# OpenDriveLab/ThinkTwice

Hardware: AMD Instinct MI355X
Metric: frames/sec forward (4-cam+LiDAR, thinktwice.py cfg) (higher is better)
Workload: dtype bf16x3h; 1 GPU; forward_inference thinktwice.py cfg: 8 frames x (2 sweeps x 4 cams x 448x896 + 65536-pt LiDAR), ResNet50+PAFPN+DepthNet+UNet+LSS splat, LidarNet, fusion, 5-stage decoder; parallelism=replicas x1 (no data-path collective), launch=eager launches, 3 batches in flight on alternating streams, batches_in_flight=3

## Files before the change

### include/thinktwice_hip.h

```cpp
#ifndef THINKTWICE_HIP_H
#define THINKTWICE_HIP_H

#include <stddef.h>
#include <stdint.h>

#ifdef __cplusplus
extern "C" {
#endif

#define TT_F32 0
#define TT_BF16 1
#define TT_F16 2

#define TT_ACT_NONE 0
#define TT_ACT_RELU 1
#define TT_ACT_SIGMOID 2
#define TT_ACT_GELU 3
#define TT_ACT_SOFTPLUS 4
#define TT_ACT_SOFTPLUS_CLAMP 5

const char* tt_last_error(void);
const char* tt_conv_last_kernel(void);
int tt_conv_set_trace(void* stamps_or_null);
int tt_version(void);
// ... 61 lines not shown
    int act;
    int dtype;
    int out_dtype;
    const int* gather_idx;
    const int* m_dev;
    float* splitk_ws;
    const void* weight_x3;
    const int* row_perm;
    const unsigned* row_mask;
    int splitk_slices;
    int in_pair, out_pair;
    const void* weight_h2;
    float* out2; int out2_cstride, out2_coff;
    int res1_up_h, res1_up_w;
    int res1_f32;
} tt_conv_desc;

int tt_conv2d_fwd(const tt_conv_desc* d, void* stream);
int tt_conv2d_splitk_slices(const tt_conv_desc* d);
int tt_conv2d_plan(const tt_conv_desc* d, char* label, int label_bytes);

int tt_seg_feedback_chain(const float* x, long long R, int x_stride, int K1, const float* w1, const float* scale1,
                          const float* shift1, int act1, const float* w2, const void* w2_x3, int N2, const float* scale2,
                          const float* shift2, int act2, float* out, int out_stride, int out_coff, void* stream);

typedef struct tt_chain_stage {
    const void* w; const float* bias;
    int K, Kp, N, act, in_sel;
    const float* res; int res_stride, res_coff;
    const float* side; const float* side_w; int side_stride, side_k;
// ... 362 lines not shown
```

### thinktwice_amd/build.py

```python
import os
import subprocess
import sys
from concurrent.futures import ThreadPoolExecutor

from . import _lib

HERE = os.path.dirname(os.path.abspath(__file__))
CSRC = os.path.join(HERE, "csrc")
OBJ = os.path.join(CSRC, "_obj")
LIB = os.path.join(HERE, "libthinktwice_hip.so")
HIPCC = os.environ.get("HIPCC", "/opt/rocm/bin/hipcc")
FLAGS = ["--offload-arch=gfx950", "-O3", "-std=c++17", "-fPIC", "-munsafe-fp-atomics", "-ffp-contract=off",
         "-Wno-unused-result"]


EXTRA_FLAGS = {"conv_x3_pipe.hip": ["-fno-slp-vectorize"]}


def _sources():
    return sorted(f for f in os.listdir(CSRC) if f.endswith((".hip", ".cpp")))


def _deps_mtime():
    hdrs = [os.path.join(CSRC, f) for f in os.listdir(CSRC) if f.endswith((".h", ".inc"))]
    hdrs.append(os.path.join(HERE, "..", "include", "thinktwice_hip.h"))
    hdrs.append(os.path.abspath(__file__))
    return max(os.path.getmtime(h) for h in hdrs)


def _compile(src, hdr_mtime, verbose):
    obj = os.path.join(OBJ, src + ".o")
# ... 81 lines not shown
```

### thinktwice_amd/csrc/conv_choose.cpp

```cpp
#include <stdint.h>

#include "conv_choose.h"

namespace tt {
namespace {

bool aligned16(const void* p) { return (reinterpret_cast<uintptr_t>(p) & 15) == 0; }

void set_tile(ConvChoice* c, int family, int bn, int waves_m, int waves_n, int bkb, int stages) {
    c->family = family;
    c->bn = bn;
    c->waves_m = waves_m;
    c->waves_n = waves_n;
    c->bkb = bkb;
    c->stages = stages;
}

bool choose_h2(const ConvArgs& a, ConvChoice* c) {
    if (a.gather || a.m_dev || a.ws || a.pixel_shuffle2 || a.Cin % 64 != 0 || a.KH * a.KW > 31 || a.K < 64) return false;
    static const bool pipe = env_flag("TT_H2_PIPE", true);
    if (pipe && a.Cout % 128 == 0 && a.K >= 1152) set_tile(c, CONV_H2_PIPE, 128, 4, 1, 128, 32);
    else if (a.Cout > 64) set_tile(c, CONV_H2, 128, 4, 2, 128, 32);
    else set_tile(c, CONV_H2, 64, 8, 1, 128, 33);
    return true;
// ... 104 lines not shown
    static const bool pipe = env_flag("TT_X3_PIPE", true);
    if (pipe && a.K >= 1152 && bn != 64 && x3_pipe_ok(a, bn)) {
        static const bool run3 = env_flag("TT_X3_RUN3", true);
        const bool runs = run3 && a.KW == 3 && a.KH <= 5 && a.stride == 1 && a.dil == 1 && a.pad == 1 && a.OH == a.H && a.OW == a.W &&
                          (a.N == 1 || a.in_nstride == (long long)a.H * a.W * a.in_cstride);
        set_tile(c, runs ? CONV_X3_RUN3 : CONV_X3_PIPE, bn, 4, 1, 128, 23);
    } else if (bn == 256) {
        set_tile(c, CONV_GLDS, 256, 4, 2, 128, 23);
    } else {
        set_tile(c, CONV_GLDS, bn, 8, 1, 128, 2);
    }
    if (bn == 256) c->main_rows = main_rows;
    return true;
}

bool choose_glds(const ConvArgs& a, int dtype, ConvChoice* c) {
    constexpr int min_tiles = 2;
    if (a.gather) {
        const bool cin_ok = a.Cin >= 16 && (a.Cin & (a.Cin - 1)) == 0;
        if (dtype == TT_F32 || !cin_ok || a.M < 2048 || a.Cout < 16 || a.Cout > 128) return false;
        if (a.Cout <= 32) set_tile(c, CONV_GLDS, 32, 8, 1, 128, 2);
        else if (a.Cout <= 64) set_tile(c, CONV_GLDS, 64, 8, 1, 128, 2);
        else set_tile(c, CONV_GLDS, 128, 4, 2, 128, 2);
        c->gather = true;
        return true;
    }
    if (a.m_dev || a.M < 2048 || a.Cout < 64 || a.KH * a.KW > 32) return false;
    if (dtype == TT_F32) {
        if (a.Cin % 16 != 0 || div_up(a.K, 16) < min_tiles) return false;
        if (a.Cout > 64) set_tile(c, CONV_GLDS, 128, 4, 2, 64, 3);
// ... 43 lines not shown
        if (a.ws_slices > 0) {
            const int eff = div_up(nk, div_up(nk, c->splits));
            TT_REQUIRE(a.ws_slices >= eff, "tt_conv2d_fwd: split-K workspace holds %d slices, %d needed", a.ws_slices, eff);
            c->slices = eff;
        }
    }
    return 0;
}

}

int conv_choose(const ConvArgs& a, const ConvFacts& f, ConvChoice* c) {
    *c = ConvChoice{};
    c->splits = 1;
    const bool ws = a.ws || f.assume_ws;
    if (f.weight_h2) {
        TT_REQUIRE(aligned16(f.weight_h2), "tt_conv2d_fwd: weight_h2 must be 16-byte aligned");
        TT_REQUIRE(choose_h2(a, c), "tt_conv2d_fwd: weight_h2 layer outside the h2 kernel's contract (Cin=%d KH*KW=%d)", a.Cin,
                   a.KH * a.KW);
        return 0;
    }
    TT_REQUIRE(!f.out2 || a.vec_epi, "tt_conv2d_fwd: out2 needs the vector epilogue (aligned channel counts)");
    TT_REQUIRE(!f.res1_up || a.vec_epi, "tt_conv2d_fwd: an upsampled res1 needs the vector epilogue (aligned channel counts)");
    TT_REQUIRE(!f.res1_f32 || (a.vec_epi && a.res_vec), "tt_conv2d_fwd: an f32 res1 needs the vector epilogue and aligned residual rows");
    TT_REQUIRE(!(f.dtype == TT_F32 && a.out_dtype != TT_F32 && a.res1) || (a.vec_epi && a.res_vec),
               "tt_conv2d_fwd: a 16-bit output of an f32 layer with a residual needs the vector epilogue");
    if (a.flags & (32 | 64)) {
        TT_REQUIRE(a.vec_epi && aligned16(f.weight_x3) && a.K % 16 == 0,
                   "tt_conv2d_fwd: in_pair / out_pair need the vector epilogue and a 16-byte aligned weight_x3");
        TT_REQUIRE(choose_x3(a, c), "tt_conv2d_fwd: pair-format layer outside the LDS-DMA bf16x3 kernel's contract (M=%d Cin=%d Cout=%d)",
// ... 23 lines not shown
    return t;
}

void conv_label(const ConvChoice& c, int dtype, char* out, size_t bytes) {
    const char* tn = dtype == TT_F32 ? "float" : "16-bit";
    const char* pre = c.apair ? " pre-split A" : "";
    const char* tail = c.main_rows > 0 ? " + tail" : "";
    switch (c.family) {
        case CONV_H2: snprintf(out, bytes, "conv_h2_kernel<%d, %d, %d, %d, %d>", c.bn, c.waves_m, c.waves_n, c.stages / 10, c.stages % 10); break;
        case CONV_H2_PIPE: snprintf(out, bytes, "conv_h2_pipe_kernel"); break;
        case CONV_SMALL: snprintf(out, bytes, "conv_small_kernel"); break;
        case CONV_SP_RUNS_L2: snprintf(out, bytes, "sp_conv_runs_l2_kernel<%d>", c.bkb / 4); break;
        case CONV_SP_RUNS: snprintf(out, bytes, "sp_conv_runs_kernel<%d, %d, %d>", c.bn / (32 * c.waves_n), c.waves_m, c.waves_n); break;
        case CONV_X3_PIPE: snprintf(out, bytes, "conv_x3_pipe_kernel<%s>%s%s", c.bn == 128 ? "4, 1, 128" : "4, 1", pre, tail); break;
        case CONV_X3_RUN3: snprintf(out, bytes, "conv_x3_run3_kernel<%d>%s%s", c.bn, pre, tail); break;
        case CONV_GLDS:
            snprintf(out, bytes, "conv_igemm_glds_kernel<%s, %d, %d, %d, %d, %d, %s, %s>%s%s", tn, c.bn, c.waves_m, c.waves_n, c.bkb,
                     c.stages, c.gather ? "true" : "false", c.x3 ? "true" : "false", pre, c.splits > 1 ? " split-K" : tail);
            break;
        default: snprintf(out, bytes, "conv_igemm_kernel<%s, 128, %d>%s", tn, c.bn, c.splits > 1 ? " split-K" : ""); break;
    }
}

}
```

### thinktwice_amd/csrc/conv_choose.h

```cpp
#pragma once
#include <stddef.h>

#include "tt_common.h"

namespace tt {

struct ConvArgs {
    const void* in;
    const void* weight;
    void* out;
    const float* scale;
    const float* shift;
    const float* shift_n;
    const void* res1;
    const void* res2;
    const int* gather;
    const int* m_dev;
    const int* row_perm;
    const unsigned* row_mask;
    float* ws;
    long long in_nstride, out_nstride;
    int N, H, W, Cin, in_cstride, in_coff;
    int Cout, KH, KW, stride, pad, dil;
    int OH, OW, out_cstride, out_coff;
// ... 12 lines not shown
    int flags;
    int res1_up_h, res1_up_w;
    float* out2;
    int out2_cstride, out2_coff;
    long long* trace;
};

enum ConvFamily {
    CONV_H2,
    CONV_H2_PIPE,
    CONV_SMALL,
    CONV_SP_RUNS_L2,
    CONV_SP_RUNS,
    CONV_X3_PIPE,
    CONV_X3_RUN3,
    CONV_GLDS,
    CONV_IGEMM,
};

constexpr int kSpL2MinRows = 16384;

struct ConvFacts {
    int dtype;
    const void* weight_x3;
    const void* weight_h2;
    bool out2, res1_up, res1_f32;
    bool assume_ws;
};

struct ConvChoice {
// ... 15 lines not shown
```

### thinktwice_amd/csrc/conv_common.h

```cpp
#pragma once
#include <type_traits>
#include "conv_choose.h"

namespace tt {
extern thread_local char g_conv_kernel[96];
extern long long* g_conv_trace;


typedef float f32x16 __attribute__((ext_vector_type(16)));
typedef __bf16 bf16x8 __attribute__((ext_vector_type(8)));
typedef _Float16 f16x8 __attribute__((ext_vector_type(8)));

template <typename T> struct Mfma;
template <> struct Mfma<float> {
    __device__ static __forceinline__ void run(const uint4& a, const uint4& b, f32x16& c) {
        c = __builtin_amdgcn_mfma_f32_32x32x2f32(__uint_as_float(a.x), __uint_as_float(b.x), c, 0, 0, 0);
        c = __builtin_amdgcn_mfma_f32_32x32x2f32(__uint_as_float(a.y), __uint_as_float(b.y), c, 0, 0, 0);
        c = __builtin_amdgcn_mfma_f32_32x32x2f32(__uint_as_float(a.z), __uint_as_float(b.z), c, 0, 0, 0);
        c = __builtin_amdgcn_mfma_f32_32x32x2f32(__uint_as_float(a.w), __uint_as_float(b.w), c, 0, 0, 0);
    }
};
template <> struct Mfma<uint16_t> {
    __device__ static __forceinline__ void run(const uint4& a, const uint4& b, f32x16& c) {
        c = __builtin_amdgcn_mfma_f32_32x32x16_bf16(__builtin_bit_cast(bf16x8, a),
// ... 381 lines not shown
            if (p.out_dtype == TT_F32)
                reinterpret_cast<float*>(p.out)[o] = v;
            else
                store16(p.out, o, v, p.out_dtype);
            if (p.out2) p.out2[(long long)mo * p.out2_cstride + p.out2_coff + co] = v;
        }
    }
}

int launch_conv_h2(const ConvChoice& c, ConvArgs& a, hipStream_t st);
int launch_conv_small(ConvArgs& a, int dtype, hipStream_t st);
int launch_sp_conv_l2(const ConvChoice& c, ConvArgs& a, hipStream_t st);
int launch_sp_conv_runs(const ConvChoice& c, ConvArgs& a, hipStream_t st);
int launch_conv_x3_pipe(const ConvChoice& c, ConvArgs& a, hipStream_t st);
int launch_conv_glds(const ConvChoice& c, ConvArgs& a, int dtype, hipStream_t st);

}
```

### thinktwice_amd/csrc/conv_igemm.hip

```cpp
#include <stdlib.h>

#include "conv_common.h"

namespace tt {

template <typename T, int BM, int BN, int WAVES_M, int WAVES_N, bool GATHER, int KX = 1>
__global__ __launch_bounds__(256) void conv_igemm_kernel(const ConvArgs p) {
    constexpr int VEC = Elem<T>::kVec;
    constexpr int BKB = ((sizeof(T) == 4) ? 64 : 128) * KX;
    constexpr int BK = BKB / (int)sizeof(T);
    constexpr int VPR = BKB / 16;
    constexpr int ROWB = BKB + 16;
    constexpr int NVA = (BM * VPR + 255) / 256;
    constexpr int NVB = (BN * VPR + 255) / 256;
    constexpr int WTM = BM / WAVES_M, WTN = BN / WAVES_N;
    constexpr int TM = WTM / 32, TN = WTN / 32;
    static_assert(WAVES_M * WAVES_N == 4, "4 waves");

    extern __shared__ __attribute__((aligned(16))) unsigned char smem[];
    const int nbuf = (p.K > BK) ? 2 : 1;
    unsigned char* sA = smem;
    unsigned char* sB = smem + nbuf * BM * ROWB;

    const int tid = threadIdx.x;
// ... 305 lines not shown
               "tt_conv2d_fwd: residuals are not supported with pixel_shuffle2");
    a.tiles_n = 1; a.cin_fast = 0; a.m_begin = 0;
    a.trace = g_conv_trace;
    a.flags = 16;
    if (d->in_pair || d->out_pair) {
        TT_REQUIRE(d->dtype == TT_F32 && d->out_dtype == TT_F32 && d->weight_x3 && !d->gather_idx && !d->splitk_ws && !d->pixel_shuffle2,
                   "tt_conv2d_fwd: in_pair / out_pair go with dense bf16x3 layers (f32 containers, weight_x3, no split-K workspace)");
        TT_REQUIRE(!d->out_pair || (!d->res1 && !d->res2 && !d->shift_n && d->Cout % 16 == 0 && d->out_cstride % 16 == 0 &&
                                    d->out_coff % 16 == 0 && (reinterpret_cast<uintptr_t>(d->out) & 63) == 0),
                   "tt_conv2d_fwd: out_pair needs Cout / out_cstride / out_coff multiples of 16, a 64-byte aligned output and no "
                   "residual / per-image shift");
        if (d->in_pair) a.flags |= 32;
        if (d->out_pair) a.flags |= 64;
    }
    if (d->res1_f32) a.flags |= 128;
    {
        const int co_vec = (d->out_dtype == TT_F32 && !d->out_pair) ? 4 : 8;
        const int osz = d->out_dtype == TT_F32 ? 4 : 2;
        const int cr = d->pixel_shuffle2 ? d->Cout / 4 : d->Cout;
        bool ok = (cr % co_vec == 0) && (d->out_cstride % co_vec == 0) && (d->out_coff % co_vec == 0) &&
                  (a.out_nstride % co_vec == 0) && ((reinterpret_cast<uintptr_t>(d->out) & 15) == 0);
        (void)osz;
        a.vec_epi = ok ? 1 : 0;
        auto res_ok = [&](const void* r, int cs, int co_) {
            return !r || ((cs % co_vec == 0) && (co_ % co_vec == 0) && ((reinterpret_cast<uintptr_t>(r) & 15) == 0));
        };
        a.res_vec = (res_ok(d->res1, d->res1_cstride, d->res1_coff) && res_ok(d->res2, d->res2_cstride, d->res2_coff)) ? 1 : 0;
    }
    f.dtype = d->dtype;
    f.weight_x3 = d->weight_x3;
// ... 28 lines not shown
            r = launch_conv_small(a, d->dtype, st);
            break;
        case CONV_SP_RUNS_L2:
            what = "tt_conv2d_fwd(sp l2)";
            r = launch_sp_conv_l2(c, a, st);
            break;
        case CONV_SP_RUNS:
            what = "tt_conv2d_fwd(glds x3)";
            r = launch_sp_conv_runs(c, a, st);
            break;
        case CONV_X3_PIPE:
        case CONV_X3_RUN3:
            what = pair ? "tt_conv2d_fwd(glds x3, pair)" : "tt_conv2d_fwd(glds x3)";
            r = launch_conv_x3_pipe(c, a, st);
            break;
        case CONV_GLDS:
            what = !c.x3 ? "tt_conv2d_fwd(glds)" : c.splits > 1 ? "tt_conv2d_fwd(glds x3 split-K)" : pair ? "tt_conv2d_fwd(glds x3, pair)" : "tt_conv2d_fwd(glds x3)";
            if (c.splits > 1) a.ws_slices = c.slices;
            r = launch_conv_glds(c, a, d->dtype, st);
            break;
        default:
            a.row_perm = nullptr;
            a.row_mask = nullptr;
            r = launch_conv_igemm(c, a, d->dtype, st);
            break;
    }
    if (r < 0) return r;
    conv_label(c, d->dtype, g_conv_kernel, sizeof(g_conv_kernel));
    if (c.main_rows > 0) {
        ConvArgs t = a;
        t.m_begin = c.main_rows * 256;
        if (launch_conv_glds(conv_tail_choice(c), t, d->dtype, st) < 0) return -1;
    }
    if (c.splits > 1) launch_splitk_finalize(a, d->dtype, st);
    return check_launch(what);
}

extern "C" int tt_conv2d_splitk_slices(const tt_conv_desc* d) {
    ConvArgs a;
    ConvFacts f;
    ConvChoice c;
    if (conv2d_prepare(d, a, f)) return 0;
    if (d->in_pair || d->out_pair || d->weight_h2 || d->res1_up_w > 0) return 0;
    f.assume_ws = true;
    if (conv_choose(a, f, &c)) return 0;
    return c.splits > 1 ? c.slices : 0;
}

extern "C" int tt_conv2d_plan(const tt_conv_desc* d, char* label, int label_bytes) {
    ConvArgs a;
    ConvFacts f;
    ConvChoice c;
    if (const int r = conv2d_prepare(d, a, f)) return r;
    if (const int r = conv_choose(a, f, &c)) return r;
    TT_REQUIRE(label && label_bytes > 0, "tt_conv2d_plan: no room for the label");
    conv_label(c, d->dtype, label, (size_t)label_bytes);
    return 0;
}
// ... 1 lines not shown
```

### thinktwice_amd/csrc/elementwise.hip

```cpp
#include "tt_common.h"

namespace tt {

template <typename T> struct Vec;
template <> struct Vec<float> {
    static constexpr int N = 4;
    float v[4];
    __device__ __forceinline__ void load(const float* p) {
        const float4 t = *reinterpret_cast<const float4*>(p);
        v[0] = t.x; v[1] = t.y; v[2] = t.z; v[3] = t.w;
    }
    __device__ __forceinline__ void store(float* p) const {
        *reinterpret_cast<float4*>(p) = make_float4(v[0], v[1], v[2], v[3]);
    }
};
template <typename T16> struct Vec16 {
    static constexpr int N = 8;
    float v[8];
    __device__ __forceinline__ void load(const T16* p) {
        const uint4 t = *reinterpret_cast<const uint4*>(p);
        const uint32_t w[4] = {t.x, t.y, t.z, t.w};
#pragma unroll
        for (int i = 0; i < 4; ++i) Pair16<T16>::unpack(w[i], v[2 * i], v[2 * i + 1]);
    }
// ... 132 lines not shown
        b.load(base + ((long long)y0 * W + x1) * C);
        cc.load(base + ((long long)y1 * W + x0) * C);
        d.load(base + ((long long)y1 * W + x1) * C);
#pragma unroll
        for (int k = 0; k < V; ++k) {
            const float top = (1.f - lx) * a.v[k] + lx * b.v[k];
            const float bot = (1.f - lx) * cc.v[k] + lx * d.v[k];
            o.v[k] = (1.f - ly) * top + ly * bot;
        }
        o.store(out + i * V);
    }
}

__global__ void bilinear_up2_ac_pair_kernel(const float* __restrict__ in, float* __restrict__ out, int N, int H, int W, int C) {
    const int cv = C / 8, OH = 2 * H, OW = 2 * W;
    const float sh = (OH > 1) ? (float)(H - 1) / (float)(OH - 1) : 0.f;
    const float sw = (OW > 1) ? (float)(W - 1) / (float)(OW - 1) : 0.f;
    const long long total = (long long)N * OH * OW * cv;
    TT_GRID_STRIDE(i, total) {
        const int c = (int)(i % cv);
        long long r = i / cv;
        const int ox = (int)(r % OW); r /= OW;
        const int oy = (int)(r % OH);
        const long long n = r / OH;
        const float fy = sh * oy, fx = sw * ox;
        const int y0 = (int)fy, x0 = (int)fx;
        const int y1 = min(y0 + 1, H - 1), x1 = min(x0 + 1, W - 1);
        const float ly = fy - y0, lx = fx - x0;
        const float* base = in + n * H * W * C + c * 8;
        float v[8];
#pragma unroll
        for (int h = 0; h < 2; ++h) {
            Vec<float> a, b, cc, d;
            a.load(base + ((long long)y0 * W + x0) * C + 4 * h);
            b.load(base + ((long long)y0 * W + x1) * C + 4 * h);
            cc.load(base + ((long long)y1 * W + x0) * C + 4 * h);
            d.load(base + ((long long)y1 * W + x1) * C + 4 * h);
#pragma unroll
            for (int k = 0; k < 4; ++k) {
                const float top = (1.f - lx) * a.v[k] + lx * b.v[k];
                const float bot = (1.f - lx) * cc.v[k] + lx * d.v[k];
                v[4 * h + k] = (1.f - ly) * top + ly * bot;
            }
        }
        uint32_t hi[4], lo[4];
#pragma unroll
        for (int e = 0; e < 4; ++e) {
            hi[e] = pack_bf16x2(v[2 * e], v[2 * e + 1]);
            lo[e] = pack_bf16x2(v[2 * e] - __uint_as_float(hi[e] << 16), v[2 * e + 1] - __uint_as_float(hi[e] & 0xffff0000u));
        }
        float* g = out + (i / cv) * C + (c >> 1) * 16 + (c & 1) * 4;
        *reinterpret_cast<uint4*>(g) = make_uint4(hi[0], hi[1], hi[2], hi[3]);
        *reinterpret_cast<uint4*>(g + 8) = make_uint4(lo[0], lo[1], lo[2], lo[3]);
    }
}

template <typename T>
__global__ __launch_bounds__(256) void spatial_pool_kernel(const T* __restrict__ in, float* __restrict__ out,
                                                           int HW, int C, int cstride, int coff, int mode) {
    const int n = blockIdx.y;
    const int c = blockIdx.x * 64 + (threadIdx.x & 63);
    const int part = threadIdx.x >> 6;
    float s = 0.f, m = -INFINITY;
    if (c < C) {
        const T* base = in + (long long)n * HW * cstride + coff + c;
        int p = part;
        for (; p + 28 < HW; p += 32) {
            float v[8];
// ... 352 lines not shown
```

### thinktwice_amd/lss.py

```python
import os

import torch

from . import _lib, camera, layers, ops, weights
from .layers import conv_from_sd, conv_from_weight, deconv2x2_from_sd, linear_from_sd, rows, unrows
from .registry import BACKBONES, NECKS, build_neck


class _ResNet50:

    def __init__(self, sd, p, dtype, device):
        vec = weights.vec_of(dtype)
        self.cin_pad = vec
        self.stem = conv_from_sd(sd, p + ".conv1", dtype, device, bn=p + ".bn1", stride=2, pad=3, act="relu",
                                 cin_pad=vec)
        self.stem_rr, self.stem_rr_x3 = None, None
        if weights.storage_dtype(dtype) != torch.float32:
            w = sd[p + ".conv1.weight"].to(device)
            wr = torch.zeros(w.shape[0], 7, 1, 64, dtype=dtype, device=device)
            wr[:, :, 0, :56] = torch.nn.functional.pad(w.permute(0, 2, 3, 1), (0, 5)).reshape(w.shape[0], 7, 56).to(dtype)
            self.stem_rr = wr.contiguous()
        elif dtype == weights.X3 and os.environ.get("TT_X3_STEM_ROWRUN", "1") == "1":
            w = sd[p + ".conv1.weight"].to(device).float()
            wr = torch.zeros(w.shape[0], 7, 1, 32, dtype=torch.float32, device=device)
# ... 340 lines not shown
    def _seg_net(self, bufs):
        cat2, cat3, cat4, e4 = bufs
        self.up["unet_layer4"](e4, out=cat4, out_coff=0)
        d4 = self.upc["unet_layer4"](cat4)
        self.up["unet_layer3"](d4, out=cat3, out_coff=0)
        d3 = self.upc["unet_layer3"](cat3)
        self.up["unet_layer2"](d3, out=cat2, out_coff=0)
        d2 = self.upc["unet_layer2"](cat2)
        from . import autodiff
        NI, h2, w2, _ = d2.shape
        H, W = 2 * h2, 2 * w2
        fused = autodiff.TAPE is None and not layers.BN_TRAIN and self.dtype == torch.float32
        x3 = self.u0a.w_x3 is not None
        p_up = x3 and ops.pair_ok(NI * H * W, 128, 64)
        p_mid = fused and x3 and self.seg_fused.w_x3 is not None and ops.pair_ok(NI * H * W, 64, self.seg_fused.w.shape[0])
        d1 = self.u0a(ops.bilinear_up2(d2, out_pair=p_up), in_pair=p_up, out_pair=p_mid)
        seg = torch.zeros(NI, H, W, self.seg_cp, dtype=self.dtype, device=d1.device)
        if fused:
            self.seg_fused(d1, out=seg, in_pair=p_mid)
        else:
            self.conv_last(self.u0b(d1), out=seg)
        return seg

    def geometry(self, gm, batch_size, num_cams):
        return ops.frustum_voxel_index(self._frustum_dev, gm, self.grid.lower, self.grid.voxel_size.tolist(),
                                       batch_size, num_cams)

    @staticmethod
    def host_constants(img_metas, num_cams=4):
        mats = camera.stack_img_metas(img_metas, num_cams)
        return {"gm": camera.geometry_matrices(mats, -1), "mlp_in": camera.depth_mlp_input(mats),
# ... 81 lines not shown
```

### thinktwice_amd/ops.py

```python
import ctypes
import os

import torch

from . import _lib
from ._lib import (TT_BF16, TT_F16, TT_F32, TTError, check, clear_device_faults, cur_stream, device_faults, lib, ptr,
                   raise_on_device_fault, require_cuda)


def dtype_code(t):
    if t.dtype == torch.float32:
        return TT_F32
    if t.dtype == torch.bfloat16:
        return TT_BF16
    if t.dtype == torch.float16:
        return TT_F16
    raise _lib.TTError(f"unsupported dtype {t.dtype}")


def frustum_voxel_index(frustum, mats, voxel_lo, voxel_size, batch_size, num_cams, want_f32=False):
    require_cuda(frustum, mats)
    assert frustum.is_contiguous() and mats.is_contiguous()
    D, fH, fW, _ = frustum.shape
    geom = torch.empty(batch_size, num_cams * D * fH * fW, 3, dtype=torch.int32, device=frustum.device)
# ... 58 lines not shown
        ("in_cstride", ctypes.c_int), ("in_coff", ctypes.c_int), ("in_nstride", ctypes.c_longlong),
        ("weight", ctypes.c_void_p), ("Cout", ctypes.c_int), ("KH", ctypes.c_int), ("KW", ctypes.c_int),
        ("stride", ctypes.c_int), ("pad", ctypes.c_int), ("dil", ctypes.c_int),
        ("out", ctypes.c_void_p), ("OH", ctypes.c_int), ("OW", ctypes.c_int), ("out_cstride", ctypes.c_int),
        ("out_coff", ctypes.c_int), ("out_nstride", ctypes.c_longlong),
        ("pixel_shuffle2", ctypes.c_int),
        ("scale", ctypes.c_void_p), ("shift", ctypes.c_void_p),
        ("shift_n", ctypes.c_void_p), ("shift_n_mod", ctypes.c_int),
        ("res1", ctypes.c_void_p), ("res1_cstride", ctypes.c_int), ("res1_coff", ctypes.c_int),
        ("res2", ctypes.c_void_p), ("res2_cstride", ctypes.c_int), ("res2_coff", ctypes.c_int),
        ("act", ctypes.c_int), ("dtype", ctypes.c_int), ("out_dtype", ctypes.c_int),
        ("gather_idx", ctypes.c_void_p), ("m_dev", ctypes.c_void_p), ("splitk_ws", ctypes.c_void_p),
        ("weight_x3", ctypes.c_void_p), ("row_perm", ctypes.c_void_p), ("row_mask", ctypes.c_void_p),
        ("splitk_slices", ctypes.c_int), ("in_pair", ctypes.c_int), ("out_pair", ctypes.c_int),
        ("weight_h2", ctypes.c_void_p), ("out2", ctypes.c_void_p), ("out2_cstride", ctypes.c_int), ("out2_coff", ctypes.c_int),
        ("res1_up_h", ctypes.c_int), ("res1_up_w", ctypes.c_int), ("res1_f32", ctypes.c_int),
    ]


def _last_conv_kernel():
    L = lib()
    return L.tt_conv_last_kernel().decode()


SPARSE_PAIRS = None


def sp_tile_plan(nbr, m_dev):
    require_cuda(nbr, m_dev)
    M, KV = nbr.shape
    ws_bytes = int(lib().tt_sp_tile_plan_workspace_bytes(M))
# ... 81 lines not shown
        autodiff.TAPE.sp_to_dense(x, coords, rows, max_rows, dims, dense)
    return dense


def sp_from_dense(gdense, coords, rows, max_rows, dims, grows):
    D, H, W = dims
    C = grows.shape[1]
    check(lib().tt_sp_from_dense(ptr(gdense), ptr(coords), ptr(rows), max_rows, C, D, H, W,
                                 ptr(grows), cur_stream(grows.device)), "tt_sp_from_dense")


def conv2d(x, w, *, stride=1, pad=0, dil=1, scale=None, shift=None, act=0, res1=None, res1_coff=0,
           res2=None, res2_coff=0, out=None, out_coff=0, in_coff=0, cin=None, pixel_shuffle2=False,
           shift_n=None, shift_n_mod=1, out_dtype=None, out_nstride=0, out_hw=None, splitk_ws=None,
           in_cstride=None, w_x3=None, _no_tape=False, stop_grad=False, bn_raw=False, in_pair=False, out_pair=False,
           w_h2=None, out2=None, out2_coff=0, res1_up=False):
    require_cuda(x, w)
    assert w.is_contiguous() and x.dim() == 4 and w.dim() == 4
    N, H, W, Cs = x.shape
    assert x.stride(3) == 1 and (W == 1 or x.stride(2) == Cs) and (H == 1 or x.stride(1) == W * Cs), x.stride()
    Cout, KH, KW, Cin = w.shape
    if cin is None:
        cin = Cin
    assert cin == Cin, (cin, Cin)
    OH = (H + 2 * pad - dil * (KH - 1) - 1) // stride + 1
    OW = (W + 2 * pad - dil * (KW - 1) - 1) // stride + 1
    if out_hw is not None:
        OH, OW = out_hw
    cr = Cout // 4 if pixel_shuffle2 else Cout
    if out is None:
        odt = out_dtype or x.dtype
        oh, ow = (2 * OH, 2 * OW) if pixel_shuffle2 else (OH, OW)
        out = torch.empty(N, oh, ow, cr, dtype=odt, device=x.device)
    d = _ConvDesc()
    d.in_ = x.data_ptr(); d.N = N; d.H = H; d.W = W; d.Cin = Cin; d.in_cstride = in_cstride or Cs; d.in_coff = in_coff
# ... 15 lines not shown
    from . import autodiff
    if w_h2 is not None:
        assert x.dtype == torch.float16 and w.dtype == torch.float16 and w_h2.dtype == torch.float16 and w_h2.is_contiguous() \
            and w_h2.numel() == 2 * w.numel() and w_x3 is None and splitk_ws is None
        if autodiff.TAPE is not None:
            raise _lib.TTError("conv2d: half-storage (h2) layers have no backward; train in dtype torch.float32 or 'f32x3'")
        d.weight_h2 = w_h2.data_ptr()
    if out2 is not None:
        assert out2.dtype == torch.float32 and out2.numel() // out2.shape[-1] == N * OH * OW and out2.stride(-1) == 1
        d.out2 = out2.data_ptr(); d.out2_cstride = out2.shape[-1]; d.out2_coff = out2_coff
    if in_pair or out_pair:
        assert w_x3 is not None and x.dtype == torch.float32 and out.dtype == torch.float32 and splitk_ws is None
        if autodiff.TAPE is not None:
            raise _lib.TTError("conv2d: pair-format activations are an inference-path layout (the tape reads f32 tensors)")
        d.in_pair, d.out_pair = int(bool(in_pair)), int(bool(out_pair))
    if w_x3 is not None and Cout < 64 and (autodiff.TAPE is not None or _no_tape):
        w_x3 = None
    if w_x3 is not None:
        assert x.dtype == torch.float32 and w_x3.shape == w.shape and w_x3.is_contiguous()
        x3_splitk = autodiff.TAPE is None and not _no_tape
        if x3_splitk:
            d.weight_x3 = w_x3.data_ptr()
    if _AUTO_SPLITK and splitk_ws is None and not (in_pair or out_pair) and w_h2 is None and not res1_up and N * OH * OW <= 4096 and KH * KW * Cin >= 2048:
        slices = int(lib().tt_conv2d_splitk_slices(ctypes.byref(d)))
        if slices > 0:
            splitk_ws = torch.empty(slices, N * OH * OW, Cout, dtype=torch.float32, device=x.device)
            d.splitk_slices = slices
    if splitk_ws is not None:
        d.splitk_ws = splitk_ws.data_ptr()
    elif w_x3 is not None:
        d.weight_x3 = w_x3.data_ptr()
    if CONV_PROFILE is not None:
        e0, e1 = torch.cuda.Event(enable_timing=True), torch.cuda.Event(enable_timing=True)
        e0.record()
    rc = lib().tt_conv2d_fwd(ctypes.byref(d), cur_stream(x.device))
    check(rc, "tt_conv2d_fwd")
    if CONV_PROFILE is not None:
        e1.record()
        CONV_PROFILE.append((2.0 * N * OH * OW * Cout * KH * KW * Cin, e0, e1,
                             f"M={N * OH * OW} N={Cout} K={KH * KW * Cin} k{KH}x{KW}s{stride}"))
        if CONV_KERNELS is not None:
            CONV_KERNELS.append(_last_conv_kernel())
        if CONV_BYTES is not None:
            esz, osz = x.element_size(), out.element_size()
            m_out = N * OH * OW
            in_px = min(N * H * W, m_out * KH * KW)
            wsz = w.numel() * w.element_size() * (2 if w_h2 is not None else 1)
            CONV_BYTES.append(in_px * (in_cstride or Cin) * esz + m_out * Cout * osz + wsz +
                              m_out * Cout * esz * ((res1 is not None) + (res2 is not None)) +
                              (m_out * Cout * 4 if out2 is not None else 0))
    if not _no_tape:
        from . import autodiff
        if autodiff.TAPE is not None:
            autodiff.TAPE.conv(x, w, out, stride, pad, dil, scale, shift, act, in_coff, cin, out_coff, res1, res1_coff,
                               res2, res2_coff, pixel_shuffle2, in_cstride, shift_n, shift_n_mod, stop_grad, bn_raw)
    return out


SEG_CHAIN = os.environ.get("TT_SEG_CHAIN", "1") != "0"


# ... 185 lines not shown
    check(lib().tt_upsample_nearest_add(ptr(dst), ptr(src), N, H, W, C, src.shape[1],
                                        src.shape[2], dtype_code(dst), _st(dst)), "tt_upsample_nearest_add")
    from . import autodiff
    if autodiff.TAPE is not None:
        autodiff.TAPE.upsample_nearest_add_(dst, src)
    return dst


PAIR = os.environ.get("TT_X3_PAIR", "1") != "0"


def pair_ok(rows, cin=32, cout=64, taps=9):
    from . import autodiff
    return (PAIR and autodiff.TAPE is None and rows > 4096 and cin % 32 == 0 and taps * cin >= 64 and
            (8 <= cout <= 32 or cout >= 64))


def bilinear_up2(x, out_pair=False):
    N, H, W, C = x.shape
    out = torch.empty(N, 2 * H, 2 * W, C, dtype=x.dtype, device=x.device)
    if out_pair:
        assert x.dtype == torch.float32 and x.is_contiguous() and C % 16 == 0
        check(lib().tt_bilinear_up2_pair(ptr(x), ptr(out), N, H, W, C, _st(x)), "tt_bilinear_up2_pair")
        return out
    check(lib().tt_bilinear_up2(ptr(x), ptr(out), N, H, W, C, dtype_code(x), _st(x)), "tt_bilinear_up2")
    from . import autodiff
    if autodiff.TAPE is not None:
        autodiff.TAPE.bilinear_up2(x, out)
    return out

# ... 633 lines not shown
```

Measured before the change: 108.4 frames/s.

## Fuse bilinear 2x upsample into the following bf16x3 3x3 conv's input patch load

Adds a dedicated conv kernel that builds its LDS input patch by bilinearly interpolating the half-resolution f32 source on the fly and splitting it into bf16 hi/lo pairs. The seg decoder's u0a layer then uses it instead of a separate bilinear_up2 kernel writing a full-resolution intermediate. This removes one kernel launch plus a write and re-read of the upsampled tensor. In exchange each patch pixel is interpolated from four source reads inside the conv, and the new kernel has a fixed tile shape and a narrow contract (Cout 64, 3x3, stride 1).

```diff
diff --git a/include/thinktwice_hip.h b/include/thinktwice_hip.h
--- a/include/thinktwice_hip.h
+++ b/include/thinktwice_hip.h
@@ -99,6 +99,7 @@
     float* out2; int out2_cstride, out2_coff;
     int res1_up_h, res1_up_w;
     int res1_f32;
+    int in_up2;
 } tt_conv_desc;
 
 int tt_conv2d_fwd(const tt_conv_desc* d, void* stream);
diff --git a/thinktwice_amd/build.py b/thinktwice_amd/build.py
--- a/thinktwice_amd/build.py
+++ b/thinktwice_amd/build.py
@@ -14,7 +14,7 @@
          "-Wno-unused-result"]
 
 
-EXTRA_FLAGS = {"conv_x3_pipe.hip": ["-fno-slp-vectorize"]}
+EXTRA_FLAGS = {"conv_x3_pipe.hip": ["-fno-slp-vectorize"], "conv_x3_up2.hip": ["-fno-slp-vectorize"]}
 
 
 def _sources():
diff --git a/thinktwice_amd/csrc/bilinear_up2.h b/thinktwice_amd/csrc/bilinear_up2.h
--- /dev/null
+++ b/thinktwice_amd/csrc/bilinear_up2.h
@@ -0,0 +1,51 @@
+#pragma once
+#include "tt_common.h"
+
+namespace tt {
+
+struct Up2Tap {
+    int y0, y1, x0, x1;
+    float ly, lx;
+};
+__device__ __forceinline__ Up2Tap up2_tap(int H, int W, int oy, int ox) {
+    const int OH = 2 * H, OW = 2 * W;
+    const float sh = (OH > 1) ? (float)(H - 1) / (float)(OH - 1) : 0.f;
+    const float sw = (OW > 1) ? (float)(W - 1) / (float)(OW - 1) : 0.f;
+    const float fy = sh * oy, fx = sw * ox;
+    Up2Tap t;
+    t.y0 = (int)fy;
+    t.x0 = (int)fx;
+    t.y1 = min(t.y0 + 1, H - 1);
+    t.x1 = min(t.x0 + 1, W - 1);
+    t.ly = fy - t.y0;
+    t.lx = fx - t.x0;
+    return t;
+}
+
+__device__ __forceinline__ void up2_pair8(const float* p00, const float* p01, const float* p10, const float* p11, float ly, float lx,
+                                          uint4& hi, uint4& lo) {
+    float v[8];
+#pragma unroll
+    for (int h = 0; h < 2; ++h) {
+        const float4 a4 = *reinterpret_cast<const float4*>(p00 + 4 * h), b4 = *reinterpret_cast<const float4*>(p01 + 4 * h);
+        const float4 c4 = *reinterpret_cast<const float4*>(p10 + 4 * h), d4 = *reinterpret_cast<const float4*>(p11 + 4 * h);
+        const float a[4] = {a4.x, a4.y, a4.z, a4.w}, b[4] = {b4.x, b4.y, b4.z, b4.w};
+        const float c[4] = {c4.x, c4.y, c4.z, c4.w}, d[4] = {d4.x, d4.y, d4.z, d4.w};
+#pragma unroll
+        for (int k = 0; k < 4; ++k) {
+            const float top = (1.f - lx) * a[k] + lx * b[k];
+            const float bot = (1.f - lx) * c[k] + lx * d[k];
+            v[4 * h + k] = (1.f - ly) * top + ly * bot;
+        }
+    }
+    uint32_t hw[4], lw[4];
+#pragma unroll
+    for (int e = 0; e < 4; ++e) {
+        hw[e] = pack_bf16x2(v[2 * e], v[2 * e + 1]);
+        lw[e] = pack_bf16x2(v[2 * e] - __uint_as_float(hw[e] << 16), v[2 * e + 1] - __uint_as_float(hw[e] & 0xffff0000u));
+    }
+    hi = make_uint4(hw[0], hw[1], hw[2], hw[3]);
+    lo = make_uint4(lw[0], lw[1], lw[2], lw[3]);
+}
+
+}
diff --git a/thinktwice_amd/csrc/conv_choose.cpp b/thinktwice_amd/csrc/conv_choose.cpp
--- a/thinktwice_amd/csrc/conv_choose.cpp
+++ b/thinktwice_amd/csrc/conv_choose.cpp
@@ -142,6 +142,26 @@
     return true;
 }
 
+int choose_up2(const ConvArgs& a, const ConvFacts& f, ConvChoice* c) {
+    TT_REQUIRE(f.dtype == TT_F32 && a.out_dtype == TT_F32 && f.weight_x3 && aligned16(f.weight_x3) && !f.weight_h2,
+               "tt_conv2d_fwd: in_up2 goes with a bf16x3 layer (f32 storage, a 16-byte aligned weight_x3)");
+    TT_REQUIRE(!a.gather && !a.m_dev && !a.ws && !a.pixel_shuffle2 && !(a.flags & 32) && !a.res1 && !a.res2 && !a.shift_n && !f.out2,
+               "tt_conv2d_fwd: in_up2 takes no in_pair, residual, per-image shift, out2, split-K workspace, gather or pixel shuffle");
+    TT_REQUIRE(a.KH == 3 && a.KW == 3 && a.stride == 1 && a.pad == 1 && a.dil == 1 && a.H % 2 == 0 && a.W % 2 == 0 && a.OH == a.H &&
+                   a.OW == a.W,
+               "tt_conv2d_fwd: in_up2 is a 3 x 3 / stride 1 / pad 1 layer over an even H x W (got %d x %d, k %d x %d s %d p %d d %d)", a.H,
+               a.W, a.KH, a.KW, a.stride, a.pad, a.dil);
+    TT_REQUIRE(a.Cin % 32 == 0 && a.Cout == 64 && a.M > 4096 && a.vec_epi,
+               "tt_conv2d_fwd: in_up2 layer outside the kernel's contract (Cin %% 32 == 0, Cout == 64, more than 4096 rows, aligned "
+               "output: M=%d Cin=%d Cout=%d)", a.M, a.Cin, a.Cout);
+    const long long img = (long long)(a.H / 2) * (a.W / 2) * a.Cin;
+    TT_REQUIRE(a.in_cstride == a.Cin && a.in_coff == 0 && a.in_nstride == img && img < (1ll << 30),
+               "tt_conv2d_fwd: in_up2 reads a contiguous [N][H/2][W/2][Cin] source of less than 2^30 elements per image");
+    set_tile(c, CONV_X3_UP2, 64, 8, 1, 128, 3);
+    c->x3 = true;
+    return 0;
+}
+
 bool choose_glds(const ConvArgs& a, int dtype, ConvChoice* c) {
     constexpr int min_tiles = 2;
     if (a.gather) {
@@ -215,6 +235,7 @@
     *c = ConvChoice{};
     c->splits = 1;
     const bool ws = a.ws || f.assume_ws;
+    if (a.flags & 256) return choose_up2(a, f, c);
     if (f.weight_h2) {
         TT_REQUIRE(aligned16(f.weight_h2), "tt_conv2d_fwd: weight_h2 must be 16-byte aligned");
         TT_REQUIRE(choose_h2(a, c), "tt_conv2d_fwd: weight_h2 layer outside the h2 kernel's contract (Cin=%d KH*KW=%d)", a.Cin,
@@ -268,6 +289,7 @@
         case CONV_SP_RUNS: snprintf(out, bytes, "sp_conv_runs_kernel<%d, %d, %d>", c.bn / (32 * c.waves_n), c.waves_m, c.waves_n); break;
         case CONV_X3_PIPE: snprintf(out, bytes, "conv_x3_pipe_kernel<%s>%s%s", c.bn == 128 ? "4, 1, 128" : "4, 1", pre, tail); break;
         case CONV_X3_RUN3: snprintf(out, bytes, "conv_x3_run3_kernel<%d>%s%s", c.bn, pre, tail); break;
+        case CONV_X3_UP2: snprintf(out, bytes, "conv_x3_run3_kernel<%d, up2>", c.bn); break;
         case CONV_GLDS:
             snprintf(out, bytes, "conv_igemm_glds_kernel<%s, %d, %d, %d, %d, %d, %s, %s>%s%s", tn, c.bn, c.waves_m, c.waves_n, c.bkb,
                      c.stages, c.gather ? "true" : "false", c.x3 ? "true" : "false", pre, c.splits > 1 ? " split-K" : tail);
diff --git a/thinktwice_amd/csrc/conv_choose.h b/thinktwice_amd/csrc/conv_choose.h
--- a/thinktwice_amd/csrc/conv_choose.h
+++ b/thinktwice_amd/csrc/conv_choose.h
@@ -50,6 +50,7 @@
     CONV_SP_RUNS,
     CONV_X3_PIPE,
     CONV_X3_RUN3,
+    CONV_X3_UP2,
     CONV_GLDS,
     CONV_IGEMM,
 };
diff --git a/thinktwice_amd/csrc/conv_common.h b/thinktwice_amd/csrc/conv_common.h
--- a/thinktwice_amd/csrc/conv_common.h
+++ b/thinktwice_amd/csrc/conv_common.h
@@ -419,5 +419,6 @@
 int launch_sp_conv_runs(const ConvChoice& c, ConvArgs& a, hipStream_t st);
 int launch_conv_x3_pipe(const ConvChoice& c, ConvArgs& a, hipStream_t st);
 int launch_conv_glds(const ConvChoice& c, ConvArgs& a, int dtype, hipStream_t st);
-
-}
+int launch_conv_x3_up2(const ConvChoice& c, ConvArgs& a, hipStream_t st);
+
+}
diff --git a/thinktwice_amd/csrc/conv_igemm.hip b/thinktwice_amd/csrc/conv_igemm.hip
--- a/thinktwice_amd/csrc/conv_igemm.hip
+++ b/thinktwice_amd/csrc/conv_igemm.hip
@@ -343,6 +343,11 @@
         if (d->out_pair) a.flags |= 64;
     }
     if (d->res1_f32) a.flags |= 128;
+    if (d->in_up2) {
+        TT_REQUIRE(!d->in_pair, "tt_conv2d_fwd: in_up2 reads an f32 source: it does not go with in_pair");
+        a.in_nstride = d->in_nstride ? d->in_nstride : (long long)(d->H / 2) * (d->W / 2) * d->in_cstride;
+        a.flags |= 256;
+    }
     {
         const int co_vec = (d->out_dtype == TT_F32 && !d->out_pair) ? 4 : 8;
         const int osz = d->out_dtype == TT_F32 ? 4 : 2;
@@ -401,6 +406,10 @@
             what = pair ? "tt_conv2d_fwd(glds x3, pair)" : "tt_conv2d_fwd(glds x3)";
             r = launch_conv_x3_pipe(c, a, st);
             break;
+        case CONV_X3_UP2:
+            what = "tt_conv2d_fwd(x3 up2)";
+            r = launch_conv_x3_up2(c, a, st);
+            break;
         case CONV_GLDS:
             what = !c.x3 ? "tt_conv2d_fwd(glds)" : c.splits > 1 ? "tt_conv2d_fwd(glds x3 split-K)" : pair ? "tt_conv2d_fwd(glds x3, pair)" : "tt_conv2d_fwd(glds x3)";
             if (c.splits > 1) a.ws_slices = c.slices;
@@ -428,7 +437,7 @@
     ConvFacts f;
     ConvChoice c;
     if (conv2d_prepare(d, a, f)) return 0;
-    if (d->in_pair || d->out_pair || d->weight_h2 || d->res1_up_w > 0) return 0;
+    if (d->in_pair || d->out_pair || d->in_up2 || d->weight_h2 || d->res1_up_w > 0) return 0;
     f.assume_ws = true;
     if (conv_choose(a, f, &c)) return 0;
     return c.splits > 1 ? c.slices : 0;
diff --git a/thinktwice_amd/csrc/conv_x3_up2.hip b/thinktwice_amd/csrc/conv_x3_up2.hip
--- /dev/null
+++ b/thinktwice_amd/csrc/conv_x3_up2.hip
@@ -0,0 +1,191 @@
+#include "bilinear_up2.h"
+#include "conv_lds_dma.h"
+
+namespace tt {
+
+namespace up2 {
+constexpr int TH = 8, TW = 32;
+constexpr int PH = TH + 2, PW = TW + 2;
+constexpr int ROWB = 128, BK = 32;
+constexpr int NT = 512, NW = 8;
+constexpr int ITEMS = PH * PW * 4, ROUNDS = (ITEMS + NT - 1) / NT;
+constexpr int PATCH_BYTES = PH * PW * ROWB;
+constexpr int W_BYTES = 64 * ROWB, W_SLOTS = 3;
+constexpr int W_OFF = PATCH_BYTES;
+constexpr int LOOP_BYTES = PATCH_BYTES + W_SLOTS * W_BYTES;
+constexpr int EPI_BYTES = NW * 32 * (64 + 4) * 4;
+constexpr int LDS_BYTES = LOOP_BYTES > EPI_BYTES ? LOOP_BYTES : EPI_BYTES;
+static_assert(ROUNDS == 3, "three production rounds per chunk");
+static_assert(2 * LDS_BYTES <= 160 * 1024, "two workgroups per CU: one's patch production runs beside the other's MFMAs");
+static_assert(2 * PW * ROWB < 65536 && W_SLOTS * W_BYTES < 65536, "tap and ring-slot shifts are ds_read offsets (16 bits)");
+}
+
+template <int OFF>
+__device__ __forceinline__ u32x4 lds_read_at(unsigned addr) {
+    u32x4 v;
+    asm volatile("ds_read_b128 %0, %1 offset:%2" : "=v"(v) : "v"(addr), "n"(OFF) : "memory");
+    return v;
+}
+
+__global__ __launch_bounds__(up2::NT, 4) void conv_x3_up2_kernel(const ConvArgs p, const void* zero_page, int tiles, int ,
+                                                                 int tiles_x, int tiles_y) {
+#if defined(__HIP_DEVICE_COMPILE__)
+    using namespace up2;
+    extern __shared__ __attribute__((aligned(16))) unsigned char smem[];
+    const int tid = threadIdx.x, lane = tid & 63, wave = tid >> 6;
+    if ((int)blockIdx.x >= tiles) return;
+    const int L = xcd_tile(tiles);
+    const int tpi = tiles_x * tiles_y;
+    const int n = L / tpi, trem = L - n * tpi;
+    const int tile_y = trem / tiles_x, tile_x = trem - tile_y * tiles_x;
+    const int oy0 = tile_y * TH, ox0 = tile_x * TW;
+    const int OH = p.OH, OW = p.OW, h = OH >> 1, w = OW >> 1, C = p.Cin;
+
+    const float* __restrict__ img = reinterpret_cast<const float*>(p.in) + (long long)n * h * w * C;
+    const float* __restrict__ wgt = reinterpret_cast<const float*>(p.weight);
+    const float* zp = reinterpret_cast<const float*>(zero_page);
+    const unsigned lds_base = (unsigned)(uintptr_t)(__attribute__((address_space(3))) unsigned char*)smem;
+    const int wave_s = __builtin_amdgcn_readfirstlane(wave);
+
+    unsigned it_off[ROUNDS];
+    unsigned it_dst[ROUNDS];
+    float it_ly[ROUNDS], it_lx[ROUNDS];
+#pragma unroll
+    for (int r = 0; r < ROUNDS; ++r) {
+        const int item = tid + NT * r;
+        const bool valid = item < ITEMS;
+        const int pix = valid ? item >> 2 : 0, g = item & 3;
+        const int py = pix / PW, px = pix - py * PW;
+        const int oy = oy0 - 1 + py, ox = ox0 - 1 + px;
+        const bool inside = valid && oy >= 0 && oy < OH && ox >= 0 && ox < OW;
+        const Up2Tap t = up2_tap(h, w, inside ? oy : 0, inside ? ox : 0);
+        it_off[r] = (unsigned)((t.y0 * w + t.x0) * C + g * 8) * 4u;
+        it_ly[r] = t.ly;
+        it_lx[r] = t.lx;
+        const unsigned dst = (unsigned)(py * PW * ROWB) + frag_off<ROWB>(px, 4u * (g >> 1) + (g & 1));
+        it_dst[r] = dst | (t.x1 != t.x0 ? 1u : 0u) | (t.y1 != t.y0 ? 2u : 0u) | (inside ? 4u : 0u);
+        if (valid && !inside) {
+            *reinterpret_cast<uint4*>(smem + dst) = make_uint4(0u, 0u, 0u, 0u);
+            *reinterpret_cast<uint4*>(smem + (dst ^ 32u)) = make_uint4(0u, 0u, 0u, 0u);
+        }
+    }
+    const unsigned dxB = (unsigned)C * 4u, dyB = (unsigned)(w * C) * 4u;
+    auto produce = [&](int ci) {
+        const char* cb = reinterpret_cast<const char*>(img + ci);
+#pragma unroll
+        for (int r = 0; r < ROUNDS; ++r) {
+            unsigned d = it_dst[r], o00 = it_off[r];
+            asm volatile("" : "+v"(d), "+v"(o00));
+            if (d & 4u) {
+                const unsigned o01 = o00 + ((d & 1u) ? dxB : 0u);
+                const unsigned o10 = o00 + ((d & 2u) ? dyB : 0u), o11 = o10 + ((d & 1u) ? dxB : 0u);
+                uint4 hi, lo;
+                up2_pair8(reinterpret_cast<const float*>(cb + o00), reinterpret_cast<const float*>(cb + o01),
+                          reinterpret_cast<const float*>(cb + o10), reinterpret_cast<const float*>(cb + o11), it_ly[r], it_lx[r], hi, lo);
+                *reinterpret_cast<uint4*>(smem + (d & ~15u)) = hi;
+                *reinterpret_cast<uint4*>(smem + ((d & ~15u) ^ 32u)) = lo;
+            }
+        }
+    };
+
+    const float* b_ptr;
+    {
+        const int g = wave * 64 + lane;
+        const int row = g >> 3, pos = g & 7;
+        b_ptr = wgt + (long long)row * p.K + (pos ^ swz<ROWB>(row)) * 4;
+    }
+    const int nch = C / BK, nk = nch * 9;
+    int w_kt = 0, w_tap = 0;
+    long long w_off = 0;
+    auto issue_w = [&](int slot) {
+        dma_piece(w_kt < nk ? b_ptr + w_off : zp, lds_base + (unsigned)(W_OFF + slot * W_BYTES) + (unsigned)wave_s * 1024u);
+        ++w_kt;
+        if (++w_tap == 9) {
+            w_tap = 0;
+            w_off += BK - 8ll * C;
+        } else {
+            w_off += C;
+        }
+    };
+
+    const unsigned hf = lane >> 5;
+    unsigned fa[3];
+#pragma unroll
+    for (int kw = 0; kw < 3; ++kw) fa[kw] = lds_base + (unsigned)(wave * PW * ROWB) + frag_off<ROWB>((lane & 31) + kw, hf);
+    const unsigned fb = lds_base + (unsigned)W_OFF + frag_off<ROWB>(lane & 31, hf);
+
+    f32x16 acc[1][2];
+    zero_acc(acc);
+
+    issue_w(0);
+    issue_w(1);
+    auto mfma_k = [&](const u32x4& ah, const u32x4& al, const u32x4 (&bh)[2], const u32x4 (&bl)[2]) {
+        const uint4 ahv = __builtin_bit_cast(uint4, ah), alv = __builtin_bit_cast(uint4, al);
+#pragma unroll
+        for (int j = 0; j < 2; ++j) Mfma<uint16_t>::run(alv, __builtin_bit_cast(uint4, bh[j]), acc[0][j]);
+#pragma unroll
+        for (int j = 0; j < 2; ++j) Mfma<uint16_t>::run(ahv, __builtin_bit_cast(uint4, bl[j]), acc[0][j]);
+#pragma unroll
+        for (int j = 0; j < 2; ++j) Mfma<uint16_t>::run(ahv, __builtin_bit_cast(uint4, bh[j]), acc[0][j]);
+    };
+    auto tap = [&](auto t_c) {
+        constexpr int t = decltype(t_c)::value;
+        constexpr int kh = t / 3, kw = t % 3, slot = t % 3;
+        constexpr int OA = kh * PW * ROWB, OB = slot * W_BYTES;
+        wait_vmcnt<1>();
+        asm volatile("s_waitcnt lgkmcnt(0)\n\ts_barrier" ::: "memory");
+        issue_w((t + 2) % 3);
+        u32x4 ah[2], al[2], bh[2][2], bl[2][2];
+        auto read_k = [&](int kc) {
+            const unsigned a = fa[kw] ^ (kc ? 64u : 0u), b = fb ^ (kc ? 64u : 0u);
+            ah[kc] = lds_read_at<OA>(a);
+            al[kc] = lds_read_at<OA>(a ^ 32u);
+            bh[kc][0] = lds_read_at<OB>(b);
+            bl[kc][0] = lds_read_at<OB>(b ^ 32u);
+            bh[kc][1] = lds_read_at<OB + 32 * ROWB>(b);
+            bl[kc][1] = lds_read_at<OB + 32 * ROWB>(b ^ 32u);
+        };
+        auto landed = [&](int kc) {
+            asm volatile("" : "+v"(ah[kc]), "+v"(al[kc]), "+v"(bh[kc][0]), "+v"(bl[kc][0]), "+v"(bh[kc][1]), "+v"(bl[kc][1]));
+        };
+        read_k(0);
+        asm volatile("s_waitcnt lgkmcnt(0)" ::: "memory");
+        read_k(1);
+        landed(0);
+        mfma_k(ah[0], al[0], bh[0], bl[0]);
+        asm volatile("s_waitcnt lgkmcnt(0)" ::: "memory");
+        landed(1);
+        mfma_k(ah[1], al[1], bh[1], bl[1]);
+    };
+    for (int c = 0; c < nch; ++c) {
+        if (c > 0) asm volatile("s_waitcnt lgkmcnt(0)\n\ts_barrier" ::: "memory");
+        produce(c * BK);
+        tap(std::integral_constant<int, 0>{});
+        tap(std::integral_constant<int, 1>{});
+        tap(std::integral_constant<int, 2>{});
+        tap(std::integral_constant<int, 3>{});
+        tap(std::integral_constant<int, 4>{});
+        tap(std::integral_constant<int, 5>{});
+        tap(std::integral_constant<int, 6>{});
+        tap(std::integral_constant<int, 7>{});
+        tap(std::integral_constant<int, 8>{});
+    }
+    wait_vmcnt<0>();
+    const int oy = oy0 + wave;
+    const bool row_ok = oy < OH;
+    const int m0 = row_ok ? (n * OH + oy) * OW + ox0 : 0;
+    const int mlim = row_ok ? (n * OH + oy) * OW + (ox0 + TW < OW ? ox0 + TW : OW) : 0;
+    conv_epilogue<float, 1, 2, 32, 64>(p, acc, smem, wave, lane, 0, 0, m0, 0, mlim);
+#endif
+}
+
+int launch_conv_x3_up2(const ConvChoice& c, ConvArgs& a, hipStream_t st) {
+    (void)c;
+    const int tiles_x = div_up(a.OW, up2::TW), tiles_y = div_up(a.OH, up2::TH);
+    const long long tiles = (long long)a.N * tiles_x * tiles_y;
+    TT_REQUIRE(tiles < (1ll << 31), "tt_conv2d_fwd: in_up2 layer of %lld tiles", tiles);
+    return launch_lds_dma(conv_x3_up2_kernel, dim3((unsigned)tiles), dim3(up2::NT), (size_t)up2::LDS_BYTES, (size_t)up2::LDS_BYTES,
+                          "conv_x3_up2_kernel", a, st, (int)tiles, 1, 1, tiles_x, tiles_y);
+}
+
+}
diff --git a/thinktwice_amd/csrc/elementwise.hip b/thinktwice_amd/csrc/elementwise.hip
--- a/thinktwice_amd/csrc/elementwise.hip
+++ b/thinktwice_amd/csrc/elementwise.hip
@@ -1,4 +1,5 @@
 #include "tt_common.h"
+#include "bilinear_up2.h"
 
 namespace tt {
 
@@ -170,8 +171,6 @@
 
 __global__ void bilinear_up2_ac_pair_kernel(const float* __restrict__ in, float* __restrict__ out, int N, int H, int W, int C) {
     const int cv = C / 8, OH = 2 * H, OW = 2 * W;
-    const float sh = (OH > 1) ? (float)(H - 1) / (float)(OH - 1) : 0.f;
-    const float sw = (OW > 1) ? (float)(W - 1) / (float)(OW - 1) : 0.f;
     const long long total = (long long)N * OH * OW * cv;
     TT_GRID_STRIDE(i, total) {
         const int c = (int)(i % cv);
@@ -179,35 +178,14 @@
         const int ox = (int)(r % OW); r /= OW;
         const int oy = (int)(r % OH);
         const long long n = r / OH;
-        const float fy = sh * oy, fx = sw * ox;
-        const int y0 = (int)fy, x0 = (int)fx;
-        const int y1 = min(y0 + 1, H - 1), x1 = min(x0 + 1, W - 1);
-        const float ly = fy - y0, lx = fx - x0;
+        const Up2Tap t = up2_tap(H, W, oy, ox);
         const float* base = in + n * H * W * C + c * 8;
-        float v[8];
-#pragma unroll
-        for (int h = 0; h < 2; ++h) {
-            Vec<float> a, b, cc, d;
-            a.load(base + ((long long)y0 * W + x0) * C + 4 * h);
-            b.load(base + ((long long)y0 * W + x1) * C + 4 * h);
-            cc.load(base + ((long long)y1 * W + x0) * C + 4 * h);
-            d.load(base + ((long long)y1 * W + x1) * C + 4 * h);
-#pragma unroll
-            for (int k = 0; k < 4; ++k) {
-                const float top = (1.f - lx) * a.v[k] + lx * b.v[k];
-                const float bot = (1.f - lx) * cc.v[k] + lx * d.v[k];
-                v[4 * h + k] = (1.f - ly) * top + ly * bot;
-            }
-        }
-        uint32_t hi[4], lo[4];
-#pragma unroll
-        for (int e = 0; e < 4; ++e) {
-            hi[e] = pack_bf16x2(v[2 * e], v[2 * e + 1]);
-            lo[e] = pack_bf16x2(v[2 * e] - __uint_as_float(hi[e] << 16), v[2 * e + 1] - __uint_as_float(hi[e] & 0xffff0000u));
-        }
+        uint4 hi, lo;
+        up2_pair8(base + ((long long)t.y0 * W + t.x0) * C, base + ((long long)t.y0 * W + t.x1) * C,
+                  base + ((long long)t.y1 * W + t.x0) * C, base + ((long long)t.y1 * W + t.x1) * C, t.ly, t.lx, hi, lo);
         float* g = out + (i / cv) * C + (c >> 1) * 16 + (c & 1) * 4;
-        *reinterpret_cast<uint4*>(g) = make_uint4(hi[0], hi[1], hi[2], hi[3]);
-        *reinterpret_cast<uint4*>(g + 8) = make_uint4(lo[0], lo[1], lo[2], lo[3]);
+        *reinterpret_cast<uint4*>(g) = hi;
+        *reinterpret_cast<uint4*>(g + 8) = lo;
     }
 }
 
diff --git a/thinktwice_amd/lss.py b/thinktwice_amd/lss.py
--- a/thinktwice_amd/lss.py
+++ b/thinktwice_amd/lss.py
@@ -378,7 +378,10 @@
         x3 = self.u0a.w_x3 is not None
         p_up = x3 and ops.pair_ok(NI * H * W, 128, 64)
         p_mid = fused and x3 and self.seg_fused.w_x3 is not None and ops.pair_ok(NI * H * W, 64, self.seg_fused.w.shape[0])
-        d1 = self.u0a(ops.bilinear_up2(d2, out_pair=p_up), in_pair=p_up, out_pair=p_mid)
+        if (ops.SEG_UP2 and x3 and fused and d2.is_contiguous() and ops.up2_ok(NI * H * W, d2.shape[-1], self.u0a.w.shape[0])):
+            d1 = self.u0a(d2, in_up2=True, out_pair=p_mid)
+        else:
+            d1 = self.u0a(ops.bilinear_up2(d2, out_pair=p_up), in_pair=p_up, out_pair=p_mid)
         seg = torch.zeros(NI, H, W, self.seg_cp, dtype=self.dtype, device=d1.device)
         if fused:
             self.seg_fused(d1, out=seg, in_pair=p_mid)
diff --git a/thinktwice_amd/ops.py b/thinktwice_amd/ops.py
--- a/thinktwice_amd/ops.py
+++ b/thinktwice_amd/ops.py
@@ -96,7 +96,7 @@
         ("weight_x3", ctypes.c_void_p), ("row_perm", ctypes.c_void_p), ("row_mask", ctypes.c_void_p),
         ("splitk_slices", ctypes.c_int), ("in_pair", ctypes.c_int), ("out_pair", ctypes.c_int),
         ("weight_h2", ctypes.c_void_p), ("out2", ctypes.c_void_p), ("out2_cstride", ctypes.c_int), ("out2_coff", ctypes.c_int),
-        ("res1_up_h", ctypes.c_int), ("res1_up_w", ctypes.c_int), ("res1_f32", ctypes.c_int),
+        ("res1_up_h", ctypes.c_int), ("res1_up_w", ctypes.c_int), ("res1_f32", ctypes.c_int), ("in_up2", ctypes.c_int),
     ]
 
 
@@ -208,11 +208,15 @@
            res2=None, res2_coff=0, out=None, out_coff=0, in_coff=0, cin=None, pixel_shuffle2=False,
            shift_n=None, shift_n_mod=1, out_dtype=None, out_nstride=0, out_hw=None, splitk_ws=None,
            in_cstride=None, w_x3=None, _no_tape=False, stop_grad=False, bn_raw=False, in_pair=False, out_pair=False,
-           w_h2=None, out2=None, out2_coff=0, res1_up=False):
+           w_h2=None, out2=None, out2_coff=0, res1_up=False, in_up2=False):
     require_cuda(x, w)
     assert w.is_contiguous() and x.dim() == 4 and w.dim() == 4
     N, H, W, Cs = x.shape
     assert x.stride(3) == 1 and (W == 1 or x.stride(2) == Cs) and (H == 1 or x.stride(1) == W * Cs), x.stride()
+    src_px = N * H * W
+    if in_up2:
+        assert x.dtype == torch.float32 and x.is_contiguous() and w_x3 is not None and not in_pair and splitk_ws is None
+        H, W = 2 * H, 2 * W
     Cout, KH, KW, Cin = w.shape
     if cin is None:
         cin = Cin
@@ -258,6 +262,10 @@
         if autodiff.TAPE is not None:
             raise _lib.TTError("conv2d: pair-format activations are an inference-path layout (the tape reads f32 tensors)")
         d.in_pair, d.out_pair = int(bool(in_pair)), int(bool(out_pair))
+    if in_up2:
+        if autodiff.TAPE is not None:
+            raise _lib.TTError("conv2d: in_up2 is an inference-path fusion (the tape records bilinear_up2 and the convolution apart)")
+        d.in_up2 = 1
     if w_x3 is not None and Cout < 64 and (autodiff.TAPE is not None or _no_tape):
         w_x3 = None
     if w_x3 is not None:
@@ -265,7 +273,7 @@
         x3_splitk = autodiff.TAPE is None and not _no_tape
         if x3_splitk:
             d.weight_x3 = w_x3.data_ptr()
-    if _AUTO_SPLITK and splitk_ws is None and not (in_pair or out_pair) and w_h2 is None and not res1_up and N * OH * OW <= 4096 and KH * KW * Cin >= 2048:
+    if _AUTO_SPLITK and splitk_ws is None and not (in_pair or out_pair or in_up2) and w_h2 is None and not res1_up and N * OH * OW <= 4096 and KH * KW * Cin >= 2048:
         slices = int(lib().tt_conv2d_splitk_slices(ctypes.byref(d)))
         if slices > 0:
             splitk_ws = torch.empty(slices, N * OH * OW, Cout, dtype=torch.float32, device=x.device)
@@ -288,7 +296,7 @@
         if CONV_BYTES is not None:
             esz, osz = x.element_size(), out.element_size()
             m_out = N * OH * OW
-            in_px = min(N * H * W, m_out * KH * KW)
+            in_px = min(src_px, m_out * KH * KW)
             wsz = w.numel() * w.element_size() * (2 if w_h2 is not None else 1)
             CONV_BYTES.append(in_px * (in_cstride or Cin) * esz + m_out * Cout * osz + wsz +
                               m_out * Cout * esz * ((res1 is not None) + (res2 is not None)) +
@@ -504,6 +512,14 @@
     from . import autodiff
     return (PAIR and autodiff.TAPE is None and rows > 4096 and cin % 32 == 0 and taps * cin >= 64 and
             (8 <= cout <= 32 or cout >= 64))
+
+
+SEG_UP2 = os.environ.get("TT_SEG_UP2", "1") != "0"
+
+
+def up2_ok(rows, cin, cout):
+    from . import autodiff
+    return autodiff.TAPE is None and rows > 4096 and cin % 32 == 0 and cout == 64
 
 
 def bilinear_up2(x, out_pair=False):
```

Measured after the change: 111.6 frames/s (median of 6 runs). 1.03x the previous value.
